# shuoshuof/Humanoid-Real-Time-Retarget

Hardware: AMD Instinct MI355X
Metric: retargeted frames/sec + max joint-angle err vs ref, Hu humanoid @1/2/4/8 GPU (higher is better)
Workload: dtype f32; 1 GPU; VtrdynFullBodyPosRetargeter batched solve, Hu v5 target (BASELINE config 3); global_batch=262144, parallelism=dp1, input_layout=soa, input_ring_sets=3, precise_gripper=True, launch=K plain launches, step i on stream i % 2

## Files before the change

humanoid-real-time-retarget_amd/csrc/rtg_math.cuh:

```cuda
#pragma once
#include <hip/hip_runtime.h>
#include <stdint.h>

#include "rtg_crmath.h"
#include "rtg_knobs.h"

#pragma clang fp contract(off)

namespace rtg {

struct Q { float x, y, z, w; };
struct V { float x, y, z; };

#define RTG_DEV __device__ __forceinline__

RTG_DEV float ieee_sqrtf(float x) { return __builtin_sqrtf(x); }
RTG_DEV float cr_sqrt(float x)
{
    const bool tiny = x < 0x1p-96f;
    const float xs = tiny ? x * 0x1p64f : x;
    float s = __builtin_amdgcn_sqrtf(xs);
    const float sdn = __uint_as_float(__float_as_uint(s) - 1u), sup = __uint_as_float(__float_as_uint(s) + 1u);
    const float rdn = __builtin_fmaf(-sdn, s, xs), rup = __builtin_fmaf(-sup, s, xs);
    s = rdn <= 0.0f ? sdn : s;
// ... 589 lines not shown
}
RTG_DEV float exp_dof_tab(float w, float qk, const uint32_t *__restrict__ tab)
{
    const uint32_t i = __float_as_uint(w) - kAngTabLo;
    const bool in = i < kAngTabEntries;
#if RTG_EXP_NO_TABLE
    const uint32_t wd = ang_tab_word(i);
    const uint32_t word = 0x24924924u + 0u * tab[0];
#else
    const uint32_t wd = ang_tab_word(i);
    const uint32_t word = tab[in ? wd : 0u];
#endif
    const float sin_theta = cr_sqrt_nt(1.0f - w * w);
    const bool mask = fabsf(sin_theta) > 1e-5f;
    const float P = exp_angle_estimate(w);
    const uint32_t code = in ? (word >> ((i - wd * kAngTabPer) * kAngTabBits)) & ((1u << kAngTabBits) - 1u) : 0u;
    float angle = __uint_as_float(__float_as_uint(P) + code - kAngTabBias);
    if (__builtin_expect(mask && code == 0u, 0)) angle = normalize_angle(2.0f * cr_acos(w));
    return mask ? angle * (qk / sin_theta) : 0.0f;
}
struct ExpDof {
    float angle, sin_theta;
    bool mask, exact;
};
RTG_DEV uint32_t ang_tab_word_of(float w)
{
    const uint32_t i = __float_as_uint(w) - kAngTabLo;
    return i < kAngTabEntries ? ang_tab_word(i) : 0u;
}
RTG_DEV ExpDof exp_dof_word_part(float w, uint32_t word);
RTG_DEV ExpDof exp_dof_table_part(float w, const uint32_t *__restrict__ tab)
{
#if RTG_EXP_NO_TABLE
    const uint32_t word = 0x24924924u + 0u * tab[0];
#else
    const uint32_t word = tab[ang_tab_word_of(w)];
#endif
    return exp_dof_word_part(w, word);
}
RTG_DEV ExpDof exp_dof_word_part(float w, uint32_t word)
{
    const uint32_t i = __float_as_uint(w) - kAngTabLo;
    const bool in = i < kAngTabEntries;
    const uint32_t wd = ang_tab_word(i);
#if RTG_EXP_NO_TABLE
    word = 0x24924924u;
#endif
    const float sin_theta = cr_sqrt_nt(1.0f - w * w);
    const bool mask = fabsf(sin_theta) > 1e-5f;
    const float P = exp_angle_estimate(w);
    const uint32_t code = in ? (word >> ((i - wd * kAngTabPer) * kAngTabBits)) & ((1u << kAngTabBits) - 1u) : 0u;
    return ExpDof{__uint_as_float(__float_as_uint(P) + code - kAngTabBias), sin_theta, mask, mask && code == 0u};
}
RTG_DEV float exp_dof_finish(const ExpDof &e, float qk) { return e.mask ? e.angle * (qk / e.sin_theta) : 0.0f; }
__device__ __attribute__((noinline)) float exp_dof_exact(float w, float qk)
{
    const float angle = normalize_angle(2.0f * cr_acos(w));
    return angle * (qk / cr_sqrt_nt(1.0f - w * w));
}
RTG_DEV float qexp_component_tab(Q q, int k, const uint32_t *__restrict__ tab)
{
    return exp_dof_tab(q.w, k == 0 ? q.x : (k == 1 ? q.y : q.z), tab);
}

RTG_DEV float dot3(V a, V b) { return (a.x * b.x + a.y * b.y) + a.z * b.z; }
RTG_DEV float lnorm3(V a)
{
    return cr_sqrt(__builtin_fmaf(a.z, a.z, __builtin_fmaf(a.y, a.y, a.x * a.x)));
}
RTG_DEV V cross3(V a, V b)
{
    return V{__builtin_fmaf(a.y, b.z, -(a.z * b.y)), __builtin_fmaf(a.z, b.x, -(a.x * b.z)),
             __builtin_fmaf(a.x, b.y, -(a.y * b.x))};
}
RTG_DEV V vsub(V a, V b) { return V{a.x - b.x, a.y - b.y, a.z - b.z}; }
RTG_DEV V vdiv(V a, float s)
{
    const Rcp r = rcp64(s);
    return mulr_v(a, r);
}
RTG_DEV V vmul(V a, float s) { return V{s * a.x, s * a.y, s * a.z}; }
template <int N>
RTG_DEV void vunit_n(const V (&a)[N], V (&u)[N])
{
    float s[N];
#pragma unroll
    for (int i = 0; i < N; ++i) s[i] = __builtin_fmaf(a[i].z, a[i].z, __builtin_fmaf(a[i].y, a[i].y, a[i].x * a[i].x));
    NormRcp r[N];
    sqrt_clamp_rcp_n<N>(s, 0.0f, r);
    mulr_n(a, r, u);
}

RTG_DEV V proj_in_plane(V v, V n)
{
    const float nn = lnorm3(n);
    return vsub(v, vmul(n, dot3(v, n) / (nn * nn)));
}

RTG_DEV float radians_between(V v1, V v2, V n)
{
    const V in[3] = {v1, v2, n};
    V u[3];
    vunit_n<3>(in, u);
    const float c = clamp_lohi(dot3(u[0], u[1]), -1.0f, 1.0f);
    return cr_acos(c) * tsign(dot3(u[2], cross3(u[0], u[1])));
}

// ... 52 lines not shown
RTG_DEV Q axis_half_quat(int axis, float a)
{
    const float h = a / 2.0f;
    const float s = cr_sin(h), c = cr_cos(h);
    return Q{axis == 0 ? s : 0.0f, axis == 1 ? s : 0.0f, axis == 2 ? s : 0.0f, c};
}

RTG_DEV float fdiv(float a, float b)
{
    return a / b;
}
RTG_DEV float la_sqrt(float x)
{
    return cr_sqrt(x);
}
RTG_DEV float la_sqrt_nt(float x) { return cr_sqrt_nt(x); }
constexpr float kDivLo = 0x1p-47f, kDivHi = 0x1p47f;
RTG_DEV bool fdiv_in_window(float x)
{
    const float ax = fabsf(x);
    return (ax >= kDivLo) & (ax <= kDivHi);
}
template <int N>
RTG_DEV void fdiv_n_bare(const float (&a)[N], float b, float (&q)[N])
{
    float y = __builtin_amdgcn_rcpf(b);
    y = __builtin_fmaf(__builtin_fmaf(-b, y, 1.0f), y, y);
#pragma unroll
    for (int i = 0; i < N; ++i) {
        float t = a[i] * y;
#pragma unroll
        for (int k = 0; k < RTG_FDIV_CORRECTIONS; ++k) t = __builtin_fmaf(__builtin_fmaf(-b, t, a[i]), y, t);
        q[i] = t;
    }
}
template <int N>
RTG_DEV void fdiv_n(const float (&a)[N], float b, float (&q)[N])
{
#if RTG_FIT_FAST_DIV_TU
    bool ok = fdiv_in_window(b);
#pragma unroll
    for (int i = 0; i < N; ++i) ok &= fdiv_in_window(a[i]);
    fdiv_n_bare<N>(a, b, q);
    if (__builtin_expect(!ok, 0)) {
#pragma unroll
        for (int i = 0; i < N; ++i) q[i] = a[i] / b;
    }
#else
#pragma unroll
    for (int i = 0; i < N; ++i) q[i] = a[i] / b;
#endif
}
RTG_DEV float la_sign(float a, float b) { return __builtin_copysignf(fabsf(a), b); }
RTG_DEV float la_lapy2(float x, float y)
{
    const float xa = fabsf(x), ya = fabsf(y);
    const float w = fmaxf(xa, ya), z = fminf(xa, ya);
    const float r = fdiv(z, w);
    return z == 0.0f ? w : w * la_sqrt_nt(1.0f + r * r);
}
template <int NX>
RTG_DEV float la_larfg(float &alpha, float &x0, float &x1)
{
    const float safmin = 1.17549435e-38f / 5.96046448e-08f, rsafmn = 1.0f / safmin;
    float xn = NX == 1 ? fabsf(x0) : la_lapy2(x0, x1);
    float beta = -__builtin_copysignf(la_lapy2(alpha, xn), alpha);
    int knt = 0;
    if (__builtin_expect((xn == 0.0f) | (fabsf(beta) < safmin), 0)) {
        if (xn == 0.0f) return 0.0f;
        do {
            ++knt;
            x0 *= rsafmn;
            if (NX == 2) x1 *= rsafmn;
            beta *= rsafmn;
            alpha *= rsafmn;
        } while (fabsf(beta) < safmin && knt < 20);
        xn = NX == 1 ? fabsf(x0) : la_lapy2(x0, x1);
        beta = -__builtin_copysignf(la_lapy2(alpha, xn), alpha);
    }
    const float tau = fdiv(beta - alpha, beta);
    const float sc = fdiv(1.0f, alpha - beta);
    x0 *= sc;
    if (NX == 2) x1 *= sc;
    for (int j = 0; j < knt; ++j) beta *= safmin;
    alpha = beta;
    return tau;
}
RTG_DEV void la_lartg(float f, float g, float &c, float &s, float &r)
{
    const float safmin = 1.17549435e-38f, safmax = 1.0f / safmin;
    const float rtmin = 1.08420217e-19f, rtmax = 1.30438176e+19f;
    const float f1 = fabsf(f), g1 = fabsf(g);
#if RTG_FIT_FAST_DIV_TU
    const bool common = (f1 >= kDivLo) & (f1 <= kDivHi) & (g1 >= kDivLo) & (g1 <= kDivHi);
    {
        const float d = la_sqrt_nt(f * f + g * g);
        const float num[2] = {f1, g};
        float quo[2];
        fdiv_n_bare<2>(num, d, quo);
        c = quo[0];
        r = __builtin_copysignf(d, f);
        s = f < 0.0f ? -quo[1] : quo[1];
    }
#else
    const bool common = (g != 0.0f) & (f != 0.0f) & (f1 > rtmin) & (f1 < rtmax) & (g1 > rtmin) & (g1 < rtmax);
    {
        const float d = la_sqrt(f * f + g * g);
        const float quo[2] = {fdiv(f1, d), fdiv(g, d)};
        c = quo[0];
        r = __builtin_copysignf(d, f);
        s = f < 0.0f ? -quo[1] : quo[1];
    }
#endif
    if (__builtin_expect(!common, 0)) {
        if (g == 0.0f) { c = 1.0f; s = 0.0f; r = f; }
        else if (f == 0.0f) { c = 0.0f; s = __builtin_copysignf(1.0f, g); r = g1; }
#if RTG_FIT_FAST_DIV_TU
        else if ((f1 > rtmin) & (f1 < rtmax) & (g1 > rtmin) & (g1 < rtmax)) {
            const float d = la_sqrt(f * f + g * g), q = fdiv(g, d);
            c = fdiv(f1, d);
            r = __builtin_copysignf(d, f);
            s = f < 0.0f ? -q : q;
        }
#endif
        else {
            const float u = fminf(safmax, fmaxf(safmin, fmaxf(f1, g1)));
            const float fs = fdiv(f, u), gs = fdiv(g, u), d = la_sqrt(fs * fs + gs * gs);
            c = fdiv(fabsf(fs), d);
            r = __builtin_copysignf(d, f);
            s = fdiv(gs, r);
            r *= u;
        }
    }
}
RTG_DEV float la_las2_min(float f, float g, float h)
{
    const float fa = fabsf(f), ga = fabsf(g), ha = fabsf(h);
    const float fhmn = fminf(fa, ha), fhmx = fmaxf(fa, ha);
    if (fhmn == 0.0f) return 0.0f;
    if (ga < fhmx) {
        const float num[3] = {fhmn, fhmx - fhmn, ga};
        float quo[3];
        fdiv_n<3>(num, fhmx, quo);
        const float as = 1.0f + quo[0], at = quo[1];
        float au = quo[2];
        au = au * au;
        const float c = fdiv(2.0f, la_sqrt_nt(as * as + au) + la_sqrt(at * at + au));
        return fhmn * c;
    }
    const float au = fdiv(fhmx, ga);
    if (au == 0.0f) return fdiv(fhmn * fhmx, ga);
    const float num[2] = {fhmn, fhmx - fhmn};
    float quo[2];
    fdiv_n<2>(num, fhmx, quo);
    const float as = 1.0f + quo[0], at = quo[1], p = as * au, q = at * au;
    const float c = fdiv(1.0f, la_sqrt_nt(1.0f + p * p) + la_sqrt_nt(1.0f + q * q));
    const float mn = (fhmn * c) * au;
    return mn + mn;
}
RTG_DEV void la_lasv2(float f, float g, float h, float &ssmin, float &ssmax, float &snr, float &csr, float &snl,
                      float &csl)
{
    const float eps = 5.96046448e-08f;
    float ft = f, fa = fabsf(ft), ht = h, ha = fabsf(h), gt = g;
    float clt = 1.0f, crt = 1.0f, slt = 0.0f, srt = 0.0f;
    int pmax = 1;
    const bool swap = ha > fa;
    if (swap) { pmax = 3; float t = ft; ft = ht; ht = t; t = fa; fa = ha; ha = t; }
    const float ga = fabsf(gt);
    if (ga == 0.0f) { ssmin = ha; ssmax = fa; }
    else {
        bool gasmal = true;
        if (ga > fa) {
            pmax = 2;
            if (fdiv(fa, ga) < eps) {
                gasmal = false;
                ssmax = ga;
                ssmin = ha > 1.0f ? fdiv(fa, fdiv(ga, ha)) : fdiv(fa, ga) * ha;
                const float num[2] = {ht, ft};
                float quo[2];
                fdiv_n<2>(num, gt, quo);
                clt = 1.0f; slt = quo[0]; srt = 1.0f; crt = quo[1];
            }
        }
        if (gasmal) {
            const float d = fa - ha, l = d == fa ? 1.0f : fdiv(d, fa);
            const float numf[2] = {gt, ht};
            float quof[2];
            fdiv_n<2>(numf, ft, quof);
            const float m = quof[0], mm = m * m;
            float t = 2.0f - l;
            const float tt = t * t;
            const float s = la_sqrt_nt(tt + mm);
            const float r = l == 0.0f ? fabsf(m) : la_sqrt(l * l + mm);
            const float a = 0.5f * (s + r);
            ssmax = fa * a;
            if (mm == 0.0f) t = l == 0.0f ? la_sign(2.0f, ft) * la_sign(1.0f, gt) : fdiv(gt, la_sign(d, ft)) + fdiv(m, t);
            else t = (fdiv(m, s + t) + fdiv(m, r + l)) * (1.0f + a);
            const float l2 = la_sqrt_nt(t * t + 4.0f);
            const float numl[2] = {2.0f, t};
            float quol[2];
            fdiv_n<2>(numl, l2, quol);
            crt = quol[0];
            srt = quol[1];
            const float numa[3] = {ha, crt + srt * m, quof[1] * srt};
            float quoa[3];
            fdiv_n<3>(numa, a, quoa);
            ssmin = quoa[0];
            clt = quoa[1];
// ... 41 lines not shown
    bool mir;
    float P, R, P2, R2;
    RTG_DEV SlotRot(bool mir_, float c, float s)
        : mir(mir_), P(mir_ ? c : s), R(mir_ ? s : c), P2(mir_ ? -s : c), R2(mir_ ? c : -s) {}
    RTG_DEV void operator()(float &lo, float &hi) const
    {
        const float Q = mir ? lo : hi, S = mir ? hi : lo;
        lo = __builtin_fmaf(P, Q, R * S);
        hi = __builtin_fmaf(P2, Q, R2 * S);
    }
};
RTG_DEV void la_bdsqr3_sort(float &d1, float &d2, float &d3, Svd3 &z)
{
    if (d1 < 0.0f) { d1 = -d1; z.vt[0] = -z.vt[0]; z.vt[3] = -z.vt[3]; z.vt[6] = -z.vt[6]; }
    if (d2 < 0.0f) { d2 = -d2; z.vt[1] = -z.vt[1]; z.vt[4] = -z.vt[4]; z.vt[7] = -z.vt[7]; }
    if (d3 < 0.0f) { d3 = -d3; z.vt[2] = -z.vt[2]; z.vt[5] = -z.vt[5]; z.vt[8] = -z.vt[8]; }
    {
        int isub = 1;
        float mn = d1;
        if (d2 <= mn) { isub = 2; mn = d2; }
        if (d3 <= mn) { isub = 3; mn = d3; }
        const bool s1 = isub == 1, s2 = isub == 2;
        d1 = s1 ? d3 : d1;
        d2 = s2 ? d3 : d2;
        d3 = mn;
#pragma unroll
        for (int k = 0; k < 3; ++k) {
            const float v0 = z.vt[3 * k], v1 = z.vt[1 + 3 * k], v2 = z.vt[2 + 3 * k];
            z.vt[3 * k] = s1 ? v2 : v0;
            z.vt[1 + 3 * k] = s2 ? v2 : v1;
            z.vt[2 + 3 * k] = s1 ? v0 : (s2 ? v1 : v2);
            const float u0 = z.u[k], u1 = z.u[k + 3], u2 = z.u[k + 6];
            z.u[k] = s1 ? u2 : u0;
            z.u[k + 3] = s2 ? u2 : u1;
            z.u[k + 6] = s1 ? u0 : (s2 ? u1 : u2);
        }
    }
    {
        const bool sw = !(d2 <= d1);
        const float t0 = d1;
        d1 = sw ? d2 : d1;
        d2 = sw ? t0 : d2;
#pragma unroll
        for (int k = 0; k < 3; ++k) {
            const float v0 = z.vt[3 * k], v1 = z.vt[1 + 3 * k];
            z.vt[3 * k] = sw ? v1 : v0;
            z.vt[1 + 3 * k] = sw ? v0 : v1;
            const float u0 = z.u[k], u1 = z.u[k + 3];
            z.u[k] = sw ? u1 : u0;
            z.u[k + 3] = sw ? u0 : u1;
        }
    }
}
RTG_DEV void la_bdsqr3(float &d1, float &d2, float &d3, float e1, float e2, Svd3 &z)
{
    const float eps = 5.96046448e-08f, tol = 10.0f * eps, unfl = 1.17549435e-38f;
    float sminoa = fabsf(d1);
    if (sminoa != 0.0f) {
        float mu = fabsf(d2) * fdiv(sminoa, sminoa + fabsf(e1));
        sminoa = fminf(sminoa, mu);
        if (sminoa != 0.0f) {
            mu = fabsf(d3) * fdiv(mu, mu + fabsf(e2));
            sminoa = fminf(sminoa, mu);
        }
    }
    sminoa = fdiv(sminoa, 1.73205078f);
    const float thresh = fmaxf(tol * sminoa, 6.0f * (3.0f * (3.0f * unfl)));
    int m = 3, iter = -1, iterdivn = 0;
    const bool mir = !(fabsf(d1) >= fabsf(d3));
    float D1 = mir ? d3 : d1, D2 = d2, D3 = mir ? d1 : d3, E1 = mir ? e2 : e1, E2 = mir ? e1 : e2;
    bool blk = false, p1 = false, run = true;
    while (run) {
        bool sweep = false;
        float shift = 0.0f;
        const float e1t = mir ? E2 : E1, e2t = mir ? E1 : E2;
        bool capped = false;
        if (iter >= 3) { iter -= 3; capped = ++iterdivn >= 18; }
        if (capped) run = false;
        else if (m == 2) {
            blk = !(fabsf(e1t) <= thresh);
            run = false;
        }
        else if (fabsf(e2t) <= thresh) m = 2;
        else if (fabsf(e1t) <= thresh) { blk = true; p1 = true; run = false; }
        else {
            const float smax = fmaxf(fmaxf(fabsf(D3), fmaxf(fabsf(D2), fabsf(E2))), fmaxf(fabsf(D1), fabsf(E1)));
            bool zeroed = false;
            float smin;
            if (fabsf(E2) <= fabsf(tol) * fabsf(D3)) { E2 = 0.0f; zeroed = true; }
            else {
                float mu = fabsf(D1);
                smin = mu;
                if (fabsf(E1) <= tol * mu) { E1 = 0.0f; zeroed = true; }
                else {
                    mu = fabsf(D2) * fdiv(mu, mu + fabsf(E1));
                    smin = fminf(smin, mu);
                    if (fabsf(E2) <= tol * mu) { E2 = 0.0f; zeroed = true; }
                    else {
                        mu = fabsf(D3) * fdiv(mu, mu + fabsf(E2));
                        smin = fminf(smin, mu);
                    }
                }
            }
            if (!zeroed) {
                sweep = true;
                if (!((3.0f * tol) * fdiv(smin, smax) <= fmaxf(eps, 0.01f * tol))) {
                    const float sll = fabsf(D1);
                    shift = la_las2_min(D2, E2, D3);
                    if (sll > 0.0f) { const float q = fdiv(shift, sll); if (q * q < eps) shift = 0.0f; }
                }
            }
        }
        if (sweep) {
            iter += 2;
            float ac, as, bc, bs, cc, cs, dc, ds;
            if (shift == 0.0f) {
                float r, h;
                la_lartg(D1, E1, ac, as, r);
                la_lartg(r, D2 * as, bc, bs, D1);
                la_lartg(D2 * ac, E2, cc, cs, r);
                E1 = bs * r;
                la_lartg(bc * r, D3 * cs, dc, ds, D2);
                h = D3 * cc;
                D3 = h * dc;
                E2 = h * ds;
            } else {
                float f = (fabsf(D1) - shift) * (__builtin_copysignf(1.0f, D1) + fdiv(shift, D1)), g = E1, r;
                la_lartg(f, g, ac, as, r);
                f = ac * D1 + as * E1;
                E1 = ac * E1 - as * D1;
                g = as * D2;
                D2 = ac * D2;
                la_lartg(f, g, bc, bs, r);
                D1 = r;
                f = bc * E1 + bs * D2;
                D2 = bc * D2 - bs * E1;
                g = bs * E2;
                E2 = bc * E2;
                la_lartg(f, g, cc, cs, r);
                E1 = r;
                f = cc * D2 + cs * E2;
                E2 = cc * E2 - cs * D2;
                g = cs * D3;
                D3 = cc * D3;
                la_lartg(f, g, dc, ds, r);
                D2 = r;
                f = dc * E2 + ds * D3;
                D3 = dc * D3 - ds * E2;
                E2 = f;
            }
            if (fabsf(E2) <= thresh) E2 = 0.0f;
            const SlotRot va(mir, mir ? bc : ac, mir ? bs : as), vc(mir, mir ? dc : cc, mir ? ds : cs);
            const SlotRot ub(mir, mir ? ac : bc, mir ? as : bs), ud(mir, mir ? cc : dc, mir ? cs : ds);
#pragma unroll
            for (int k = 0; k < 3; ++k) va(z.vt[3 * k], z.vt[1 + 3 * k]);
#pragma unroll
            for (int k = 0; k < 3; ++k) vc(z.vt[1 + 3 * k], z.vt[2 + 3 * k]);
#pragma unroll
            for (int k = 0; k < 3; ++k) ub(z.u[k], z.u[k + 3]);
#pragma unroll
            for (int k = 0; k < 3; ++k) ud(z.u[k + 3], z.u[k + 6]);
        }
    }
    d1 = mir ? D3 : D1; d2 = D2; d3 = mir ? D1 : D3;
    e1 = mir ? E2 : E1; e2 = mir ? E1 : E2;
#pragma unroll
    for (int i = 0; i < 4; ++i) {
        const float v0 = z.vt[i], v1 = z.vt[8 - i], u0 = z.u[i], u1 = z.u[8 - i];
        z.vt[i] = mir ? v1 : v0;
        z.vt[8 - i] = mir ? v0 : v1;
        z.u[i] = mir ? u1 : u0;
        z.u[8 - i] = mir ? u0 : u1;
    }
    if (blk) {
        float sigmn, sigmx, sinr, cosr, sinl, cosl;
        la_lasv2(p1 ? d2 : d1, p1 ? e2 : e1, p1 ? d3 : d2, sigmn, sigmx, sinr, cosr, sinl, cosl);
        d1 = p1 ? d1 : sigmx;
        d2 = p1 ? sigmx : sigmn;
        d3 = p1 ? sigmn : d3;
        vt_rot(z, p1, cosr, sinr);
        u_rot(z, p1, cosl, sinl);
    }
    la_bdsqr3_sort(d1, d2, d3, z);
}
struct NoHook {
    RTG_DEV void operator()(int) const {}
};
RTG_DEV void la_gebd2_rest(float a[9], float &tp0, float &tq1, float &e1, float &d2, float &e2, float &d3)
{
    float dum = 0.0f;
    tp0 = la_larfg<1>(a[3], a[6], dum);
    e1 = a[3];
    if (tp0 != 0.0f) {
        const float tv1 = -(tp0 * 1.0f), tv2 = -(tp0 * a[6]);
#pragma unroll
        for (int r = 1; r < 3; ++r) {
            const float w = __builtin_fmaf(a[r + 6], a[6], a[r + 3]);
            a[r + 3] = __builtin_fmaf(w, tv1, a[r + 3]);
            a[r + 6] = __builtin_fmaf(w, tv2, a[r + 6]);
        }
    }
    tq1 = la_larfg<1>(a[4], a[5], dum);
    d2 = a[4];
    if (tq1 != 0.0f) {
        const float w = a[7] + a[8] * a[5];
        const float tw = -(tq1 * w);
        a[7] = __builtin_fmaf(1.0f, tw, a[7]);
        a[8] = __builtin_fmaf(a[5], tw, a[8]);
    }
    e2 = a[7];
    d3 = a[8];
}
RTG_DEV void la_ormbr3(const float a[9], float tq0, float tq1, float tp0, Svd3 &z)
{
    if (tq1 != 0.0f) {
#pragma unroll
        for (int j = 0; j < 3; ++j) {
            const float w = z.u[1 + 3 * j] + z.u[2 + 3 * j] * a[5];
            const float tw = -(tq1 * w);
            z.u[1 + 3 * j] = __builtin_fmaf(-tq1, w, z.u[1 + 3 * j]);
            z.u[2 + 3 * j] = __builtin_fmaf(a[5], tw, z.u[2 + 3 * j]);
        }
    }
    if (tq0 != 0.0f) {
#pragma unroll
        for (int j = 0; j < 3; ++j) {
            const float w = z.u[3 * j] + (z.u[1 + 3 * j] * a[1] + z.u[2 + 3 * j] * a[2]);
            const float tw = -(tq0 * w);
            z.u[3 * j] = __builtin_fmaf(-tq0, w, z.u[3 * j]);
            z.u[1 + 3 * j] = __builtin_fmaf(a[1], tw, z.u[1 + 3 * j]);
            z.u[2 + 3 * j] = __builtin_fmaf(a[2], tw, z.u[2 + 3 * j]);
        }
    }
    if (tp0 != 0.0f) {
        const float tv1 = -(tp0 * 1.0f), tv2 = -(tp0 * a[6]);
#pragma unroll
        for (int r = 0; r < 3; ++r) {
            const float w = __builtin_fmaf(z.vt[r + 6], a[6], z.vt[r + 3]);
            z.vt[r + 3] = __builtin_fmaf(w, tv1, z.vt[r + 3]);
            z.vt[r + 6] = __builtin_fmaf(w, tv2, z.vt[r + 6]);
        }
    }
}
template <typename Hook = NoHook>
RTG_DEV void la_gesdd3(float a[9], Svd3 &z, const Hook &hook = Hook{})
{
    const float smlnum = 9.09494702e-13f, bignum = 1.0f / smlnum;
    float anrm = 0.0f;
#pragma unroll
    for (int i = 0; i < 9; ++i) anrm = fmaxf(anrm, fabsf(a[i]));
    if (__builtin_expect((anrm > 0.0f && anrm < smlnum) || anrm > bignum, 0)) {
        const float mul = anrm < smlnum ? fdiv(smlnum, anrm) : fdiv(bignum, anrm);
#pragma unroll
        for (int i = 0; i < 9; ++i) a[i] *= mul;
    }
    const float tq0 = la_larfg<2>(a[0], a[1], a[2]);
    const float d1 = a[0];
    if (tq0 != 0.0f) {
#pragma unroll
        for (int j = 1; j < 3; ++j) {
            const float w = a[3 * j] + (a[1 + 3 * j] * a[1] + a[2 + 3 * j] * a[2]);
            const float tw = -(tq0 * w);
            a[3 * j] = __builtin_fmaf(1.0f, tw, a[3 * j]);
            a[1 + 3 * j] = __builtin_fmaf(a[1], tw, a[1 + 3 * j]);
            a[2 + 3 * j] = __builtin_fmaf(a[2], tw, a[2 + 3 * j]);
        }
    }
    float tp0, tq1, e1, d2, e2, d3;
    la_gebd2_rest(a, tp0, tq1, e1, d2, e2, d3);
    hook(10);
#pragma unroll
    for (int i = 0; i < 9; ++i) { z.u[i] = (i % 4 == 0) ? 1.0f : 0.0f; z.vt[i] = z.u[i]; }
    float s1 = d1, s2 = d2, s3 = d3;
    la_bdsqr3(s1, s2, s3, e1, e2, z);
    hook(11);
    la_ormbr3(a, tq0, tq1, tp0, z);
}
template <typename Hook = NoHook>
RTG_DEV bool la_gesdd3_x0(float a[9], bool fin, Svd3 &z, const Hook &hook = Hook{})
{
    const float smlnum = 9.09494702e-13f, bignum = 1.0f / smlnum;
    const float eps = 5.96046448e-08f, tol = 10.0f * eps, unfl = 1.17549435e-38f;
    float anrm = 0.0f;
#pragma unroll
    for (int i = 3; i < 9; ++i) anrm = fmaxf(anrm, fabsf(a[i]));
    if (__builtin_expect((anrm > 0.0f && anrm < smlnum) || anrm > bignum, 0)) {
        const float mul = anrm < smlnum ? fdiv(smlnum, anrm) : fdiv(bignum, anrm);
#pragma unroll
        for (int i = 3; i < 9; ++i) a[i] *= mul;
    }
    float tp0, tq1, e1, d2, e2, d3;
    la_gebd2_rest(a, tp0, tq1, e1, d2, e2, d3);
    hook(10);
    const float thresh = 6.0f * (3.0f * (3.0f * unfl));
    const bool ok = fin && fabsf(e2) > thresh && fabsf(e1) > thresh && fabsf(d3) > 0.0f &&
                    !(fabsf(e2) <= tol * fabsf(d3)) && fabsf(e1) > tol * fabsf(d2);
    if (__builtin_amdgcn_ballot_w64(!ok) != 0) return false;
#pragma unroll
    for (int i = 0; i < 9; ++i) { z.u[i] = (i % 4 == 0) ? 1.0f : 0.0f; z.vt[i] = z.u[i]; }
    float ac, as, bc, bs, cc, cs, r, s3;
    la_lartg(d3, e2, ac, as, r);
    la_lartg(r, d2 * as, bc, bs, s3);
    la_lartg(d2 * ac, e1, cc, cs, r);
    float s1 = 0.0f, s2 = bc * r;
    e2 = bs * r;
    vt_rot(z, true, bc, -bs);
    vt_rot(z, false, 1.0f, -0.0f);
    u_rot(z, true, ac, -as);
    u_rot(z, false, cc, -cs);
    if (!(fabsf(e2) <= thresh)) {
        float sigmn, sigmx, sinr, cosr, sinl, cosl;
        la_lasv2(s2, e2, s3, sigmn, sigmx, sinr, cosr, sinl, cosl);
        s2 = sigmx;
        s3 = sigmn;
        vt_rot(z, true, cosr, sinr);
        u_rot(z, true, cosl, sinl);
    }
    la_bdsqr3_sort(s1, s2, s3, z);
    hook(11);
    la_ormbr3(a, 0.0f, tq1, tp0, z);
    return true;
}
RTG_DEV void kabsch_of_svd(Svd3 &z, float R[9])
{
#pragma unroll
    for (int i = 0; i < 3; ++i)
#pragma unroll
        for (int k = 0; k < 3; ++k)
            R[i * 3 + k] = (z.u[i] * z.vt[3 * k] + z.u[i + 3] * z.vt[1 + 3 * k]) + z.u[i + 6] * z.vt[2 + 3 * k];
    const float det = R[0] * (R[4] * R[8] - R[5] * R[7]) - R[1] * (R[3] * R[8] - R[5] * R[6]) +
                      R[2] * (R[3] * R[7] - R[4] * R[6]);
    if (det < 0.0f) {
#pragma unroll
        for (int k = 0; k < 3; ++k) z.vt[2 + 3 * k] = -z.vt[2 + 3 * k];
#pragma unroll
        for (int i = 0; i < 3; ++i)
#pragma unroll
            for (int k = 0; k < 3; ++k)
                R[i * 3 + k] = (z.u[i] * z.vt[3 * k] + z.u[i + 3] * z.vt[1 + 3 * k]) + z.u[i + 6] * z.vt[2 + 3 * k];
    }
}
template <typename Hook = NoHook>
RTG_DEV void kabsch_rot(const float A[9], float R[9], const Hook &hook = Hook{})
{
#if RTG_EXP_STUB_SVD
#pragma unroll
    for (int i = 0; i < 9; ++i) R[i] = (i % 4 == 0) ? 1.0f : A[i] * 1e-3f;
    return;
#endif
    float a[9];
#pragma unroll
    for (int i = 0; i < 3; ++i)
#pragma unroll
        for (int k = 0; k < 3; ++k) a[i + 3 * k] = A[i * 3 + k];
    Svd3 z;
    la_gesdd3(a, z, hook);
    kabsch_of_svd(z, R);
}

template <int N>
RTG_DEV bool form_joint_A(const V (&Z)[N], const V (&M)[N], float (&A)[9])
{
#pragma unroll
    for (int i = 0; i < 3; ++i)
#pragma unroll
        for (int k = 0; k < 3; ++k) {
            float acc = 0.0f;
#pragma unroll
            for (int j = 0; j < N; ++j) {
                const float mi = i == 0 ? M[j].x : (i == 1 ? M[j].y : M[j].z);
                const float zk = k == 0 ? Z[j].x : (k == 1 ? Z[j].y : Z[j].z);
                const float pr = mi * zk;
                acc = j == 0 ? pr : acc + pr;
            }
            A[i * 3 + k] = acc;
        }
    bool nan = false;
#pragma unroll
    for (int i = 0; i < 9; ++i) nan |= A[i] != A[i];
    return nan;
}
template <typename Hook = NoHook, typename Tab = NoTab>
RTG_DEV Q joint_quat_of_A(const float (&A)[9], const Hook &hook = Hook{}, Tab tab = Tab{})
{
    hook(0);
    float R[9];
    kabsch_rot(A, R, hook);
    hook(1);
    return qfrom_rotmat(R, tab);
}
template <typename Hook = NoHook, typename Tab = NoTab>
RTG_DEV bool torso_quat_x0(const V (&Z)[3], const V (&M)[3], Q &q, const Hook &hook = Hook{}, Tab tab = Tab{})
{
    float a[9];
    float sum = 0.0f;
#pragma unroll
    for (int i = 0; i < 3; ++i) {
#pragma unroll
        for (int j = 0; j < 3; ++j) sum += fabsf(i == 0 ? M[j].x : (i == 1 ? M[j].y : M[j].z));
#pragma unroll
        for (int k = 1; k < 3; ++k) {
            float acc = 0.0f;
#pragma unroll
            for (int j = 0; j < 3; ++j) {
                const float mi = i == 0 ? M[j].x : (i == 1 ? M[j].y : M[j].z);
                const float pr = mi * (k == 1 ? Z[j].y : Z[j].z);
                acc = j == 0 ? pr : acc + pr;
            }
            a[i + 3 * k] = acc;
        }
        a[i] = 0.0f;
    }
    hook(0);
    Svd3 z;
    if (!la_gesdd3_x0(a, sum < 0x1p60f, z, hook)) return false;
    float R[9];
    kabsch_of_svd(z, R);
    hook(1);
    q = qfrom_rotmat(R, tab);
    return true;
}
template <int N, typename Hook = NoHook, typename Tab = NoTab>
RTG_DEV Q cal_joint_quat(const V (&Z)[N], const V (&M)[N], bool &svd_nan, const Hook &hook = Hook{}, Tab tab = Tab{})
{
    float A[9];
    svd_nan = form_joint_A<N>(Z, M, A);
    return joint_quat_of_A(A, hook, tab);
}
template <int N, typename Hook = NoHook>
RTG_DEV Q cal_joint_quat(const V (&Z)[N], const V (&M)[N], const Hook &hook = Hook{})
{
    bool unused;
    return cal_joint_quat<N>(Z, M, unused, hook);
}

struct DD { double h, l; };
RTG_DEV DD dd_fast_sum(double a, double b) { const double s = a + b; return DD{s, b - (s - a)}; }
RTG_DEV DD dd_two_sum(double a, double b)
{
    const double s = a + b, bb = s - a;
    return DD{s, (a - (s - bb)) + (b - bb)};
}
RTG_DEV DD dd_two_prod(double a, double b) { const double p = a * b; return DD{p, __builtin_fma(a, b, -p)}; }
RTG_DEV DD dd_add(DD a, DD b)
{
    const DD s = dd_two_sum(a.h, b.h), t = dd_two_sum(a.l, b.l);
    const DD u = dd_fast_sum(s.h, s.l + t.h);
    return dd_fast_sum(u.h, u.l + t.l);
}
RTG_DEV DD dd_neg(DD a) { return DD{-a.h, -a.l}; }
RTG_DEV DD dd_mul(DD a, DD b)
{
    const DD p = dd_two_prod(a.h, b.h);
    return dd_fast_sum(p.h, p.l + __builtin_fma(a.h, b.l, a.l * b.h));
}
RTG_DEV DD dd_div(DD a, DD b)
{
    const double inv = 1.0 / b.h;
    const double q1 = a.h * inv;
    const DD p = dd_two_prod(q1, b.h);
    const double r = (((a.h - p.h) - p.l) + a.l) - q1 * b.l;
    return dd_fast_sum(q1, r * inv);
}
RTG_DEV DD dd_atan_tab(int k)
{
    static constexpr double T[33][2] = {
    {0x0.0p+0, 0x0.0p+0},
    {0x1.ffd55bba97625p-6, -0x1.5ec431444912cp-60},
    {0x1.ff55bb72cfdeap-5, -0x1.c934d86d23f1dp-60},
    {0x1.7ee182602f10fp-4, -0x1.cfb654c0c3d98p-58},
    {0x1.fd5ba9aac2f6ep-4, -0x1.cd37686760c17p-59},
    {0x1.3d6eee8c6626cp-3, 0x1.61a3b0ce9281bp-57},
    {0x1.7b97b4bce5b02p-3, 0x1.347b0b4f881cap-58},
    {0x1.b90d7529260a2p-3, 0x1.17b10d2e0e5abp-61},
    {0x1.f5b75f92c80ddp-3, 0x1.8ab6e3cf7afbdp-57},
    {0x1.18bf5a30bf178p-2, 0x1.30ca4748b1bf9p-57},
    {0x1.362773707ebccp-2, -0x1.963a544b672d8p-57},
    {0x1.530ad9951cd4ap-2, -0x1.2566480884082p-57},
    {0x1.6f61941e4def1p-2, -0x1.c63aae6f6e918p-56},
    {0x1.8b24d394a1b25p-2, 0x1.b6d0ba3748fa8p-56},
// ... 222 lines not shown
        vec[3 * a] = v1p;
        vec[3 * a + 1] = v1r;
        vec[3 * a + 2] = SHOULDER ? cross3(v1p, ey) : cross3(ez, v1p);
    }
    V u[3 * NA];
    vunit_n<3 * NA>(vec, u);
    float c[2 * NA];
#pragma unroll
    for (int a = 0; a < NA; ++a) {
        c[2 * a] = clamp_lohi(dot3(ex, u[3 * a]), -1.0f, 1.0f);
        c[2 * a + 1] = clamp_lohi(dot3(u[3 * a], u[3 * a + 1]), -1.0f, 1.0f);
    }
    float ac[2 * NA];
    cr_acos_n<2 * NA>(c, ac);
    float ang[2 * NA];
    V ax[2 * NA];
#pragma unroll
    for (int a = 0; a < NA; ++a) {
        ang[2 * a] = ac[2 * a] * tsign(dot3(pn, cross3(ex, u[3 * a]))) - z0[a].th0;
        ax[2 * a] = pn;
        ang[2 * a + 1] = ac[2 * a + 1] * tsign(dot3(u[3 * a + 2], cross3(u[3 * a], u[3 * a + 1]))) - z0[a].ph0;
        ax[2 * a + 1] = SHOULDER ? ex : ey;
    }
    Q q[2 * NA];
    qfrom_angle_unit_axis_n<2 * NA>(ang, ax, q, tab);
#pragma unroll
    for (int a = 0; a < NA; ++a) {
        first[a] = q[2 * a];
        second[a] = q[2 * a + 1];
    }
}
template <bool SHOULDER, typename Tab>
RTG_DEV void arm_pair_1(V v1, ArmZero z0, Q parent, Q &first, Q &second, Tab tab)
{
    const V v[1] = {v1};
    const ArmZero z[1] = {z0};
    const Q par[1] = {parent};
    Q a[1], b[1];
    arm_pair_n<SHOULDER, 1>(v, z, par, a, b, tab);
    first = a[0];
    second = b[0];
}
template <typename Tab = NoTab>
RTG_DEV void shoulder_pr(V v1, ArmZero z0, Q parent, Q &pitch, Q &roll, Tab tab = Tab{})
{
    arm_pair_1<true>(v1, z0, parent, pitch, roll, tab);
}
template <typename Tab = NoTab>
RTG_DEV void elbow_py(V v1, ArmZero z0, Q parent, Q &yaw, Q &elbow, Tab tab = Tab{})
{
    arm_pair_1<false>(v1, z0, parent, yaw, elbow, tab);
}

RTG_DEV float mean5(float v0, float v1, float v2, float v3, float v4)
{
    return ((((v0 + v4) + v1) + v2) + v3) / 5.0f;
}

__constant__ static const int8_t kHuDofAxis[30] = {2, 0, 1, 1, 1, 2, 0, 1, 1, 1, 2, 1, 0, 2, 1,
                                                   0, 1, 2, 1, 1, 1, 0, 2, 1, 0, 1, 2, 1, 1, 2};
__host__ __device__ constexpr int hu_dof_axis(int k)
{
    constexpr int8_t t[30] = {2, 0, 1, 1, 1, 2, 0, 1, 1, 1, 2, 1, 0, 2, 1,
                              0, 1, 2, 1, 1, 1, 0, 2, 1, 0, 1, 2, 1, 1, 2};
    return t[k];
}

}
```

humanoid-real-time-retarget_amd/csrc/rtg_solver.cuh:

```cuda
#pragma once
#include "rtg_device.cuh"

namespace rtg {

struct Emit {
    float *row;
    float *__restrict__ lr;
    const uint32_t *__restrict__ ang;
    float2 *st;
    int sst;
    uint32_t *wd = nullptr;
    template <int LINK>
    static constexpr int slot() { return LINK <= 18 ? LINK - 12 : LINK - 14; }
    RTG_DEV void load_word(int s, float w) const
    {
#if !RTG_EXP_NO_TABLE
        __builtin_amdgcn_global_load_lds((const __attribute__((address_space(1))) void *)(ang + ang_tab_word_of(w)),
                                         (__attribute__((address_space(3))) void *)(wd + s * 64), 4, 0, 0);
#endif
    }
    template <int LINK>
    RTG_DEV void link(Q q) const
    {
        constexpr int k = hu_dof_axis(LINK - 1);
        st[slot<LINK>() * sst] = make_float2(q.w, k == 0 ? q.x : (k == 1 ? q.y : q.z));
        if (wd) load_word(slot<LINK>(), q.w);
        if (lr) st4(lr + 4 * LINK, q);
    }
    template <int LINK>
    RTG_DEV void identity() const
    {
        st[slot<LINK>() * sst] = make_float2(1.0f, 0.0f);
        if (lr) st4(lr + 4 * LINK, qident());
    }
    RTG_DEV void finalize(int s0, int n) const
    {
        uint32_t exact = 0;
        if (wd) wait_words();
#pragma unroll
        for (int j = 0; j < 14; ++j)
            if (j >= s0 && j < s0 + n) {
                const float2 v = st[j * sst];
                const ExpDof e = wd ? exp_dof_word_part(v.x, wd[j * 64 + (threadIdx.x & 63)]) : exp_dof_table_part(v.x, ang);
                exact |= (uint32_t)e.exact << j;
                row[j < 7 ? 11 + j : 13 + j] = exp_dof_finish(e, v.y);
            }
        if (__builtin_expect(exact != 0u, 0)) {
#pragma unroll 1
            for (int j = s0; j < s0 + n; ++j)
                if ((exact >> j) & 1u) {
                    const float2 v = st[j * sst];
                    row[j < 7 ? 11 + j : 13 + j] = exp_dof_exact(v.x, v.y);
                }
        }
    }
    static RTG_DEV void wait_words() { __builtin_amdgcn_s_waitcnt(0x0F70); }
    RTG_DEV Emit shifted(int dl, int ds) const
    {
        return Emit{row + dl, lr ? lr + 4 * dl : nullptr, ang, st + ds * sst, sst, wd ? wd + ds * 64 : nullptr};
    }
};
constexpr bool side_links_alike(int a, int b, int n)
{
    for (int j = 0; j < n; ++j)
        if (hu_dof_axis(a + j - 1) != hu_dof_axis(b + j - 1)) return false;
    return true;
}

RTG_DEV void emit_fixed_links(const Emit &E, bool write_lr = true, int k0 = 0)
{
#pragma unroll
    for (int k = 0; k < 11; ++k)
        if (k >= k0) E.row[k] = 0.0f;
    E.row[29] = 0.0f;
    if (E.lr && write_lr) {
#pragma unroll
        for (int j = 0; j < 12; ++j) st4(E.lr + 4 * j, qident());
        st4(E.lr + 4 * 19, qident());
        st4(E.lr + 4 * 20, qident());
        st4(E.lr + 4 * 28, qident());
        st4(E.lr + 4 * 29, qident());
        st4(E.lr + 4 * 30, qident());
    }
}

enum : uint32_t {
    kStTorsoSvd = 1,
    kStLeftSvd = 2,
    kStLeftEuler = 4,
    kStRightSvd = 8,
    kStRightEuler = 16,
};
RTG_DEV uint32_t frame_error_code(uint32_t bits)
{
    const uint32_t first = bits & (0u - bits);
    return (first & (kStTorsoSvd | kStLeftSvd | kStRightSvd)) ? RTG_FRAME_SVD_NONFINITE : RTG_FRAME_ZERO_NORM_QUAT;
}
// ... 687 lines not shown
            const bool s0 = sub == 0, s1 = sub == 1;
            const Q e{s0 ? eul[0].x : (s1 ? eul[1].x : eul[2].x), s0 ? eul[0].y : (s1 ? eul[1].y : eul[2].y),
                      s0 ? eul[0].z : (s1 ? eul[1].z : eul[2].z), s0 ? eul[0].w : (s1 ? eul[1].w : eul[2].w)};
            if (sub < 3) link_rt(E, L0 + sub, e);
            return false;
        }
    }
    double q[4] = {(double)qf.x, (double)qf.y, (double)qf.z, (double)qf.w};
    const double nrm = sqrt(q[0] * q[0] + q[1] * q[1] + q[2] * q[2] + q[3] * q[3]);
    const bool refused = !(nrm > 0.0);
    q[0] /= nrm; q[1] /= nrm; q[2] /= nrm; q[3] /= nrm;
    const int sign = -1;
    const double qi = q[2], qj = q[1], qk = q[0];
    const double a = q[3] - qj, b = qi + qk * sign, c = qj + q[3], d = qk * sign - qi;
    double at = 0.0;
    if (sub < 3) {
        const double Y = sub == 0 ? euler_hypot(c, d) : (sub == 1 ? b : d);
        const double X = sub == 0 ? euler_hypot(a, b) : (sub == 1 ? a : c);
        at = euler_atan2(Y, X);
    }
    double ang[3];
    ang[1] = 2.0 * gbc<G, 0>(at);
    const double half_sum = gbc<G, 1>(at), half_diff = gbc<G, 2>(at);
    int kase = 0;
    if (fabs(ang[1]) <= 1e-7) kase = 1;
    else if (fabs(ang[1] - M_PI) <= 1e-7) kase = 2;
    if (kase == 0) {
        ang[0] = half_sum - half_diff;
        ang[2] = half_sum + half_diff;
    } else {
        ang[0] = 0.0;
        ang[2] = kase == 1 ? 2.0 * half_sum : 2.0 * half_diff;
    }
    ang[2] *= sign;
    ang[1] -= M_PI / 2.0;
    { const double tt = ang[0]; ang[0] = ang[2]; ang[2] = tt; }
#pragma unroll
    for (int t = 0; t < 3; ++t) {
        if (ang[t] < -M_PI) ang[t] += 2.0 * M_PI;
        else if (ang[t] > M_PI) ang[t] -= 2.0 * M_PI;
    }
    if (sub < 3) link_rt(E, L0 + sub, elementary_quat(sub, sub == 0 ? ang[0] : (sub == 1 ? ang[1] : ang[2])));
    return refused;
}
template <int G = 64>
RTG_DEV void finalize_lanes(const Emit &E, int s0, int n)
{
    const int sub = sublane<G>();
    if (sub < n) {
        const int j = s0 + sub;
        const float2 v = E.st[j * E.sst];
        const ExpDof e = exp_dof_table_part(v.x, E.ang);
        float val = exp_dof_finish(e, v.y);
        if (__builtin_expect(e.exact, 0)) val = normalize_angle(2.0f * cr_acos(v.x)) * (v.y / e.sin_theta);
        E.row[j < 7 ? 11 + j : 13 + j] = val;
    }
}

template <bool PRECISE, typename Tab = NoTab, typename TabF = NoTab>
RTG_DEV uint32_t fbp_frame1_tile(const SolverConsts &C, const float *rows, float *__restrict__ dof,
                                 float *__restrict__ local_rot, float *__restrict__ body_rot, bool const_rows = true,
                                 Tab tab = Tab{}, TabF tabF = TabF{})
{
    __shared__ float sdof[kDofStride];
    __shared__ float4 sfit, schain[2];
    __shared__ float2 sst[14];
    __shared__ int sflag[3];
    __shared__ uint32_t sstat[3];
    const int w = threadIdx.x >> 6, lane = threadIdx.x & 63;
    const bool w0 = lane == 0;
#if RTG_EXP_TIMESTAMPS
    float *const tsb = body_rot;
    body_rot = nullptr;
    auto TS = [&](int k) {
        if (tsb && lane == 0) {
            const uint64_t t = wall_clock64();
            reinterpret_cast<uint32_t *>(tsb)[2 * (16 * w + k)] = (uint32_t)t;
            reinterpret_cast<uint32_t *>(tsb)[2 * (16 * w + k) + 1] = (uint32_t)(t >> 32);
        }
    };
#else
    auto TS = [](int) {};
#endif
    auto hook = [&](int k) { TS(k == 0 ? 1 : (k == 10 ? 2 : (k == 11 ? 3 : 4))); };
    TS(0);
    if (threadIdx.x < 3) sflag[threadIdx.x] = 0;
    __syncthreads();
    const Emit E{sdof, local_rot, C.ang_tab, sst, 1};
    const FV<false> b{rows};
    uint32_t st = 0;
    Q fitq = qident();
    bool fit_nan = false;
    if (w < 3 && w0) {
        float A[9];
        if (w == 0) {
            const V b10 = b.p3(10);
            const V Mt[3] = {vsub(b.p3(17), b10), vsub(b.p3(13), b10), vsub(b.p3(11), b10)};
            fit_nan = form_joint_A<3>(C.Zt, Mt, A);
        } else {
            const FV<false> H{rows + (w == 2 ? 123 : 63)};
            const V h0 = H.p3(0);
            const V M[5] = {vsub(H.p3(2), h0), vsub(H.p3(6), h0), vsub(H.p3(10), h0), vsub(H.p3(14), h0),
                            vsub(H.p3(17), h0)};
            V Z[5];
#pragma unroll
            for (int k = 0; k < 5; ++k) Z[k] = w == 2 ? C.Zr[k] : C.Zl[k];
            fit_nan = form_joint_A<5>(Z, M, A);
// ... 301 lines not shown
```

Before: 4.640 billion frames/s.

## Use bare fast divisions with range guards in SVD, exp-dof and mean paths

Replaces IEEE divisions in several hot paths (exp-dof finish, Householder larfg, bdsqr shift computation, las2_min, division by sqrt3 and by 5) with bare reciprocal-based divisions. Each path is guarded by a range check that falls back to the exact IEEE path when operands leave a safe window. Constant divisors use a precomputed reciprocal with an FMA correction step. The aim is to cut the cost of the precise division sequences while keeping results bit-exact, at the price of more code, extra predicate checks and a possible rise in register pressure.

New measurement: 4.775 billion frames/s (median of 6 runs). 2.9% higher.

```diff
diff --git a/humanoid-real-time-retarget_amd/csrc/rtg_math.cuh b/humanoid-real-time-retarget_amd/csrc/rtg_math.cuh
--- a/humanoid-real-time-retarget_amd/csrc/rtg_math.cuh
+++ b/humanoid-real-time-retarget_amd/csrc/rtg_math.cuh
@@ -665,7 +665,13 @@
     const uint32_t code = in ? (word >> ((i - wd * kAngTabPer) * kAngTabBits)) & ((1u << kAngTabBits) - 1u) : 0u;
     return ExpDof{__uint_as_float(__float_as_uint(P) + code - kAngTabBias), sin_theta, mask, mask && code == 0u};
 }
-RTG_DEV float exp_dof_finish(const ExpDof &e, float qk) { return e.mask ? e.angle * (qk / e.sin_theta) : 0.0f; }
+RTG_DEV float fdiv1(float a, float b);
+RTG_DEV float exp_dof_finish(const ExpDof &e, float qk) { return e.mask ? e.angle * fdiv1(qk, e.sin_theta) : 0.0f; }
+RTG_DEV bool exp_dof_redo(const ExpDof &e, float qk)
+{
+    const float a = fabsf(qk);
+    return e.exact | (e.mask & !((a >= 0x1p-76f) & (a <= 0x1p47f)));
+}
 __device__ __attribute__((noinline)) float exp_dof_exact(float w, float qk)
 {
     const float angle = normalize_angle(2.0f * cr_acos(w));
@@ -824,6 +830,36 @@
 #endif
 }
 RTG_DEV float la_sign(float a, float b) { return __builtin_copysignf(fabsf(a), b); }
+constexpr float kNumLo = 0x1p-76f;
+RTG_DEV float fdiv1(float a, float b)
+{
+    const float num[1] = {a};
+    float q[1];
+    fdiv_n_bare<1>(num, b, q);
+    return q[0];
+}
+RTG_DEV bool fdiv1_in_n(float a, float b)
+{
+    const float aa = fabsf(a);
+    return fdiv_in_window(b) & (aa >= kNumLo) & (aa <= kDivHi);
+}
+constexpr float kConstNumHi = 0x1p94f;
+RTG_DEV bool fdiv1_in_c(float a)
+{
+    const float aa = fabsf(a);
+    return (aa >= kNumLo) & (aa <= kConstNumHi);
+}
+RTG_DEV float fdiv1_const(float a, float c, float y)
+{
+    const float t = a * y;
+    return __builtin_fmaf(__builtin_fmaf(-c, t, a), y, t);
+}
+template <bool BARE>
+RTG_DEV float fdiv_g(float a, float b)
+{
+    if constexpr (BARE) return fdiv1(a, b);
+    else return a / b;
+}
 RTG_DEV float la_lapy2(float x, float y)
 {
     const float xa = fabsf(x), ya = fabsf(y);
@@ -831,8 +867,14 @@
     const float r = fdiv(z, w);
     return z == 0.0f ? w : w * la_sqrt_nt(1.0f + r * r);
 }
+RTG_DEV float la_lapy2_bare(float xa, float ya)
+{
+    const float w = fmaxf(xa, ya), z = fminf(xa, ya);
+    const float r = fdiv1(z, w);
+    return z == 0.0f ? w : w * la_sqrt_nt(1.0f + r * r);
+}
 template <int NX>
-RTG_DEV float la_larfg(float &alpha, float &x0, float &x1)
+RTG_DEV float la_larfg_ieee(float &alpha, float &x0, float &x1)
 {
     const float safmin = 1.17549435e-38f / 5.96046448e-08f, rsafmn = 1.0f / safmin;
     float xn = NX == 1 ? fabsf(x0) : la_lapy2(x0, x1);
@@ -858,6 +900,31 @@
     alpha = beta;
     return tau;
 }
+template <int NX>
+RTG_DEV bool la_larfg_ok(float alpha, float x0, float x1)
+{
+    const float xa0 = fabsf(x0), w = NX == 1 ? xa0 : fmaxf(xa0, fabsf(x1));
+    return (w >= 0x1p-46f) & (w <= 0x1p45f) & (fabsf(alpha) <= 0x1p45f);
+}
+template <int NX, bool S1 = true>
+RTG_DEV float la_larfg(float &alpha, float &x0, float &x1)
+{
+#if RTG_FIT_FAST_DIV_TU
+    if constexpr (!S1) return la_larfg_ieee<NX>(alpha, x0, x1);
+    if (__builtin_expect(!la_larfg_ok<NX>(alpha, x0, x1), 0)) return la_larfg_ieee<NX>(alpha, x0, x1);
+    const float xa0 = fabsf(x0);
+    const float xn = NX == 1 ? xa0 : la_lapy2_bare(xa0, fabsf(x1));
+    const float beta = -__builtin_copysignf(la_lapy2_bare(fabsf(alpha), xn), alpha);
+    const float tau = fdiv1(beta - alpha, beta);
+    const float sc = fdiv1(1.0f, alpha - beta);
+    x0 *= sc;
+    if (NX == 2) x1 *= sc;
+    alpha = beta;
+    return tau;
+#else
+    return la_larfg_ieee<NX>(alpha, x0, x1);
+#endif
+}
 RTG_DEV void la_lartg(float f, float g, float &c, float &s, float &r)
 {
     const float safmin = 1.17549435e-38f, safmax = 1.0f / safmin;
@@ -905,6 +972,7 @@
         }
     }
 }
+template <bool BARE = false>
 RTG_DEV float la_las2_min(float f, float g, float h)
 {
     const float fa = fabsf(f), ga = fabsf(g), ha = fabsf(h);
@@ -913,20 +981,22 @@
     if (ga < fhmx) {
         const float num[3] = {fhmn, fhmx - fhmn, ga};
         float quo[3];
-        fdiv_n<3>(num, fhmx, quo);
+        if constexpr (BARE) fdiv_n_bare<3>(num, fhmx, quo);
+        else fdiv_n<3>(num, fhmx, quo);
         const float as = 1.0f + quo[0], at = quo[1];
         float au = quo[2];
         au = au * au;
-        const float c = fdiv(2.0f, la_sqrt_nt(as * as + au) + la_sqrt(at * at + au));
+        const float c = fdiv_g<BARE>(2.0f, la_sqrt_nt(as * as + au) + la_sqrt(at * at + au));
         return fhmn * c;
     }
-    const float au = fdiv(fhmx, ga);
+    const float au = fdiv_g<BARE>(fhmx, ga);
     if (au == 0.0f) return fdiv(fhmn * fhmx, ga);
     const float num[2] = {fhmn, fhmx - fhmn};
     float quo[2];
-    fdiv_n<2>(num, fhmx, quo);
+    if constexpr (BARE) fdiv_n_bare<2>(num, fhmx, quo);
+    else fdiv_n<2>(num, fhmx, quo);
     const float as = 1.0f + quo[0], at = quo[1], p = as * au, q = at * au;
-    const float c = fdiv(1.0f, la_sqrt_nt(1.0f + p * p) + la_sqrt_nt(1.0f + q * q));
+    const float c = fdiv_g<BARE>(1.0f, la_sqrt_nt(1.0f + p * p) + la_sqrt_nt(1.0f + q * q));
     const float mn = (fhmn * c) * au;
     return mn + mn;
 }
@@ -1074,19 +1144,85 @@
         }
     }
 }
-RTG_DEV void la_bdsqr3(float &d1, float &d2, float &d3, float e1, float e2, Svd3 &z)
-{
-    const float eps = 5.96046448e-08f, tol = 10.0f * eps, unfl = 1.17549435e-38f;
+constexpr float kStLo = 0x1p-46f, kStHi = 0x1p46f;
+constexpr float kSqrt3 = 1.73205078f, kRcpSqrt3 = 0x1.279a74p-1f;
+template <bool BARE>
+RTG_DEV float la_bdsqr3_sminoa(float d1, float d2, float d3, float e1, float e2)
+{
     float sminoa = fabsf(d1);
     if (sminoa != 0.0f) {
-        float mu = fabsf(d2) * fdiv(sminoa, sminoa + fabsf(e1));
+        float mu = fabsf(d2) * fdiv_g<BARE>(sminoa, sminoa + fabsf(e1));
         sminoa = fminf(sminoa, mu);
         if (sminoa != 0.0f) {
-            mu = fabsf(d3) * fdiv(mu, mu + fabsf(e2));
+            mu = fabsf(d3) * fdiv_g<BARE>(mu, mu + fabsf(e2));
             sminoa = fminf(sminoa, mu);
         }
     }
-    sminoa = fdiv(sminoa, 1.73205078f);
+    return sminoa;
+}
+struct BdsqrPass { int zero; float shift; };
+template <bool BARE>
+RTG_DEV BdsqrPass la_bdsqr3_shift(float D1, float D2, float D3, float E1, float E2, float smax)
+{
+    const float eps = 5.96046448e-08f, tol = 10.0f * eps;
+    BdsqrPass p{0, 0.0f};
+    if (fabsf(E2) <= fabsf(tol) * fabsf(D3)) p.zero = 2;
+    else {
+        float mu = fabsf(D1), smin = mu;
+        if (fabsf(E1) <= tol * mu) p.zero = 1;
+        else {
+            mu = fabsf(D2) * fdiv_g<BARE>(mu, mu + fabsf(E1));
+            smin = fminf(smin, mu);
+            if (fabsf(E2) <= tol * mu) p.zero = 2;
+            else {
+                mu = fabsf(D3) * fdiv_g<BARE>(mu, mu + fabsf(E2));
+                smin = fminf(smin, mu);
+                if (!((3.0f * tol) * fdiv_g<BARE>(smin, smax) <= fmaxf(eps, 0.01f * tol))) {
+                    const float sll = fabsf(D1), sh = la_las2_min<BARE>(D2, E2, D3);
+                    const float q = fdiv_g<BARE>(sh, sll);
+                    p.shift = ((BARE || sll > 0.0f) && q * q < eps) ? 0.0f : sh;
+                }
+            }
+        }
+    }
+    return p;
+}
+RTG_DEV bool la_bdsqr3_state_ok(float D1, float D2, float D3, float E1, float E2, float smax)
+{
+    const float smn = fminf(fminf(fabsf(D3), fminf(fabsf(D2), fabsf(E2))), fminf(fabsf(D1), fabsf(E1)));
+    return (smn >= kStLo) & (smax <= kStHi);
+}
+RTG_DEV float la_bdsqr3_smax(float D1, float D2, float D3, float E1, float E2)
+{
+    return fmaxf(fmaxf(fabsf(D3), fmaxf(fabsf(D2), fabsf(E2))), fmaxf(fabsf(D1), fabsf(E1)));
+}
+template <bool S1 = true>
+RTG_DEV BdsqrPass la_bdsqr3_pass(float D1, float D2, float D3, float E1, float E2, float smax)
+{
+#if RTG_FIT_FAST_DIV_TU
+    if (S1 && __builtin_expect(la_bdsqr3_state_ok(D1, D2, D3, E1, E2, smax), 1)) return la_bdsqr3_shift<true>(D1, D2, D3, E1, E2, smax);
+#endif
+    return la_bdsqr3_shift<false>(D1, D2, D3, E1, E2, smax);
+}
+template <bool S1 = true>
+RTG_DEV float la_bdsqr3_entry(float d1, float d2, float d3, float e1, float e2)
+{
+#if RTG_FIT_FAST_DIV_TU
+    if constexpr (!S1) return fdiv(la_bdsqr3_sminoa<false>(d1, d2, d3, e1, e2), kSqrt3);
+    const float s = la_bdsqr3_sminoa<true>(d1, d2, d3, e1, e2);
+    const bool ok = la_bdsqr3_state_ok(d1, d2, d3, e1, e2, la_bdsqr3_smax(d1, d2, d3, e1, e2)) & (s >= kNumLo);
+    float q = fdiv1_const(s, kSqrt3, kRcpSqrt3);
+    if (__builtin_expect(!ok, 0)) q = fdiv(la_bdsqr3_sminoa<false>(d1, d2, d3, e1, e2), kSqrt3);
+    return q;
+#else
+    return fdiv(la_bdsqr3_sminoa<false>(d1, d2, d3, e1, e2), kSqrt3);
+#endif
+}
+template <bool S1 = true>
+RTG_DEV void la_bdsqr3(float &d1, float &d2, float &d3, float e1, float e2, Svd3 &z)
+{
+    const float eps = 5.96046448e-08f, tol = 10.0f * eps, unfl = 1.17549435e-38f;
+    const float sminoa = la_bdsqr3_entry<S1>(d1, d2, d3, e1, e2);
     const float thresh = fmaxf(tol * sminoa, 6.0f * (3.0f * (3.0f * unfl)));
     int m = 3, iter = -1, iterdivn = 0;
     const bool mir = !(fabsf(d1) >= fabsf(d3));
@@ -1106,32 +1242,12 @@
         else if (fabsf(e2t) <= thresh) m = 2;
         else if (fabsf(e1t) <= thresh) { blk = true; p1 = true; run = false; }
         else {
-            const float smax = fmaxf(fmaxf(fabsf(D3), fmaxf(fabsf(D2), fabsf(E2))), fmaxf(fabsf(D1), fabsf(E1)));
-            bool zeroed = false;
-            float smin;
-            if (fabsf(E2) <= fabsf(tol) * fabsf(D3)) { E2 = 0.0f; zeroed = true; }
-            else {
-                float mu = fabsf(D1);
-                smin = mu;
-                if (fabsf(E1) <= tol * mu) { E1 = 0.0f; zeroed = true; }
-                else {
-                    mu = fabsf(D2) * fdiv(mu, mu + fabsf(E1));
-                    smin = fminf(smin, mu);
-                    if (fabsf(E2) <= tol * mu) { E2 = 0.0f; zeroed = true; }
-                    else {
-                        mu = fabsf(D3) * fdiv(mu, mu + fabsf(E2));
-                        smin = fminf(smin, mu);
-                    }
-                }
-            }
-            if (!zeroed) {
-                sweep = true;
-                if (!((3.0f * tol) * fdiv(smin, smax) <= fmaxf(eps, 0.01f * tol))) {
-                    const float sll = fabsf(D1);
-                    shift = la_las2_min(D2, E2, D3);
-                    if (sll > 0.0f) { const float q = fdiv(shift, sll); if (q * q < eps) shift = 0.0f; }
-                }
-            }
+            const float smax = la_bdsqr3_smax(D1, D2, D3, E1, E2);
+            const BdsqrPass ps = la_bdsqr3_pass<S1>(D1, D2, D3, E1, E2, smax);
+            E1 = ps.zero == 1 ? 0.0f : E1;
+            E2 = ps.zero == 2 ? 0.0f : E2;
+            sweep = ps.zero == 0;
+            shift = ps.shift;
         }
         if (sweep) {
             iter += 2;
@@ -1208,10 +1324,11 @@
 struct NoHook {
     RTG_DEV void operator()(int) const {}
 };
+template <bool S1 = true>
 RTG_DEV void la_gebd2_rest(float a[9], float &tp0, float &tq1, float &e1, float &d2, float &e2, float &d3)
 {
     float dum = 0.0f;
-    tp0 = la_larfg<1>(a[3], a[6], dum);
+    tp0 = la_larfg<1, S1>(a[3], a[6], dum);
     e1 = a[3];
     if (tp0 != 0.0f) {
         const float tv1 = -(tp0 * 1.0f), tv2 = -(tp0 * a[6]);
@@ -1222,7 +1339,7 @@
             a[r + 6] = __builtin_fmaf(w, tv2, a[r + 6]);
         }
     }
-    tq1 = la_larfg<1>(a[4], a[5], dum);
+    tq1 = la_larfg<1, S1>(a[4], a[5], dum);
     d2 = a[4];
     if (tq1 != 0.0f) {
         const float w = a[7] + a[8] * a[5];
@@ -1264,7 +1381,7 @@
         }
     }
 }
-template <typename Hook = NoHook>
+template <bool S1 = true, typename Hook = NoHook>
 RTG_DEV void la_gesdd3(float a[9], Svd3 &z, const Hook &hook = Hook{})
 {
     const float smlnum = 9.09494702e-13f, bignum = 1.0f / smlnum;
@@ -1276,7 +1393,7 @@
 #pragma unroll
         for (int i = 0; i < 9; ++i) a[i] *= mul;
     }
-    const float tq0 = la_larfg<2>(a[0], a[1], a[2]);
+    const float tq0 = la_larfg<2, S1>(a[0], a[1], a[2]);
     const float d1 = a[0];
     if (tq0 != 0.0f) {
 #pragma unroll
@@ -1289,12 +1406,12 @@
         }
     }
     float tp0, tq1, e1, d2, e2, d3;
-    la_gebd2_rest(a, tp0, tq1, e1, d2, e2, d3);
+    la_gebd2_rest<S1>(a, tp0, tq1, e1, d2, e2, d3);
     hook(10);
 #pragma unroll
     for (int i = 0; i < 9; ++i) { z.u[i] = (i % 4 == 0) ? 1.0f : 0.0f; z.vt[i] = z.u[i]; }
     float s1 = d1, s2 = d2, s3 = d3;
-    la_bdsqr3(s1, s2, s3, e1, e2, z);
+    la_bdsqr3<S1>(s1, s2, s3, e1, e2, z);
     hook(11);
     la_ormbr3(a, tq0, tq1, tp0, z);
 }
@@ -1362,7 +1479,7 @@
                 R[i * 3 + k] = (z.u[i] * z.vt[3 * k] + z.u[i + 3] * z.vt[1 + 3 * k]) + z.u[i + 6] * z.vt[2 + 3 * k];
     }
 }
-template <typename Hook = NoHook>
+template <bool S1 = true, typename Hook = NoHook>
 RTG_DEV void kabsch_rot(const float A[9], float R[9], const Hook &hook = Hook{})
 {
 #if RTG_EXP_STUB_SVD
@@ -1376,7 +1493,7 @@
 #pragma unroll
         for (int k = 0; k < 3; ++k) a[i + 3 * k] = A[i * 3 + k];
     Svd3 z;
-    la_gesdd3(a, z, hook);
+    la_gesdd3<S1>(a, z, hook);
     kabsch_of_svd(z, R);
 }
 
@@ -1402,12 +1519,12 @@
     for (int i = 0; i < 9; ++i) nan |= A[i] != A[i];
     return nan;
 }
-template <typename Hook = NoHook, typename Tab = NoTab>
+template <bool S1 = true, typename Hook = NoHook, typename Tab = NoTab>
 RTG_DEV Q joint_quat_of_A(const float (&A)[9], const Hook &hook = Hook{}, Tab tab = Tab{})
 {
     hook(0);
     float R[9];
-    kabsch_rot(A, R, hook);
+    kabsch_rot<S1>(A, R, hook);
     hook(1);
     return qfrom_rotmat(R, tab);
 }
@@ -1447,7 +1564,7 @@
 {
     float A[9];
     svd_nan = form_joint_A<N>(Z, M, A);
-    return joint_quat_of_A(A, hook, tab);
+    return joint_quat_of_A<N != 3>(A, hook, tab);
 }
 template <int N, typename Hook = NoHook>
 RTG_DEV Q cal_joint_quat(const V (&Z)[N], const V (&M)[N], const Hook &hook = Hook{})
@@ -1776,9 +1893,15 @@
     arm_pair_1<false>(v1, z0, parent, yaw, elbow, tab);
 }
 
+RTG_DEV float fdiv_by5(float s)
+{
+    float q = fdiv1_const(s, 5.0f, 0x1.99999ap-3f);
+    if (__builtin_expect(!fdiv1_in_c(s), 0)) q = s / 5.0f;
+    return q;
+}
 RTG_DEV float mean5(float v0, float v1, float v2, float v3, float v4)
 {
-    return ((((v0 + v4) + v1) + v2) + v3) / 5.0f;
+    return fdiv_by5(((((v0 + v4) + v1) + v2) + v3));
 }
 
 __constant__ static const int8_t kHuDofAxis[30] = {2, 0, 1, 1, 1, 2, 0, 1, 1, 1, 2, 1, 0, 2, 1,
diff --git a/humanoid-real-time-retarget_amd/csrc/rtg_solver.cuh b/humanoid-real-time-retarget_amd/csrc/rtg_solver.cuh
--- a/humanoid-real-time-retarget_amd/csrc/rtg_solver.cuh
+++ b/humanoid-real-time-retarget_amd/csrc/rtg_solver.cuh
@@ -42,7 +42,7 @@
             if (j >= s0 && j < s0 + n) {
                 const float2 v = st[j * sst];
                 const ExpDof e = wd ? exp_dof_word_part(v.x, wd[j * 64 + (threadIdx.x & 63)]) : exp_dof_table_part(v.x, ang);
-                exact |= (uint32_t)e.exact << j;
+                exact |= (uint32_t)exp_dof_redo(e, v.y) << j;
                 row[j < 7 ? 11 + j : 13 + j] = exp_dof_finish(e, v.y);
             }
         if (__builtin_expect(exact != 0u, 0)) {
@@ -836,7 +836,7 @@
         const float2 v = E.st[j * E.sst];
         const ExpDof e = exp_dof_table_part(v.x, E.ang);
         float val = exp_dof_finish(e, v.y);
-        if (__builtin_expect(e.exact, 0)) val = normalize_angle(2.0f * cr_acos(v.x)) * (v.y / e.sin_theta);
+        if (__builtin_expect(exp_dof_redo(e, v.y), 0)) val = normalize_angle(2.0f * cr_acos(v.x)) * (v.y / e.sin_theta);
         E.row[j < 7 ? 11 + j : 13 + j] = val;
     }
 }
```
